# OettlM/STEDM

Hardware: AMD Instinct MI355X
Metric: U-Net denoising steps/sec (32x32x4 latent, bs=64) (higher is better)
Workload: dtype f16; 1 GPU; HER2-style DDIM-50 + CFG 1.5 (rescale 0.7) denoising step, NS32 U-Net (234.6M params, random-init PRNG weights), 32x32x4 latents + 3-ch layout concat, style vector 512; batch_per_gpu=64, global_batch=64, latent=32x32x4, cfg=cond+uncond per step, parallelism=dp1 (independent latents, no in-loop collective)

## Files before the change

include/stedm_hip.h:

```cpp
#ifndef STEDM_HIP_H
#define STEDM_HIP_H

#include <stdint.h>

#ifdef __cplusplus
extern "C" {
#endif

#define STEDM_ABI_VERSION 12

#define STEDM_F16 0
#define STEDM_BF16 1

#define STEDM_CONV_S1 0
#define STEDM_CONV_DOWN 1
#define STEDM_CONV_UP 2
#define STEDM_CONV_UP_SUBPIXEL 3
#define STEDM_CONV_S2D 4

int stedm_abi_version(void);
const char* stedm_last_error(void);
int stedm_device_cus(void);

#define STEDM_F16G_RAW 1
// ... 90 lines not shown
  int32_t gn_only;
  void* gn_out16_lo;
  void* qkv_q;
  void* qkv_k;
  void* qkv_vt;
  int32_t qkv_T, qkv_Tp, qkv_heads;
  float qkv_qscale;
  const float* ln_gamma;
  const float* ln_beta;
  const float* ln_res;
  float ln_eps;
  int32_t out16_stride;
  void* gn_coop;
  const uint32_t* gn_coop_epoch;
  uint32_t* gn_coop_tmo;
} stedm_conv_args;
int stedm_conv_igemm(const stedm_conv_args* args, void* stream);
int stedm_conv_fused_skip_ok(const stedm_conv_args* args);
int stedm_conv3x3_tiles_ok(int Hout, int Wout);
int stedm_im2col_rows16(const void* src16, void* dst16, int B, int Hs, int Ws, int C, int mode, void* stream);
int stedm_conv_rs_ok(const stedm_conv_args* args);

int stedm_conv_in(const float* x1, int c1, const float* x2, int c2, int x2_bmod, const float* w_oihw,
                  const float* bias, float* out, int B, int H, int W, int cout, float* chan_stats, void* stream);
int stedm_conv_out(const float* src, int c, const float* chan_stats, int nslab, const float* gamma, const float* beta,
                   float eps, int groups, const float* w_hwio, const float* bias, float* out, int B, int H, int W,
                   int cout, void* stream);

int stedm_time_embed(const int64_t* t, const float* freqs, const float* w0t, const float* b0,
                     const float* w2t, const float* b2, float* emb, float* ws, int B, int mc, int ted,
// ... 135 lines not shown
```

stedm_amd/_lib.py:

```python
from __future__ import annotations

import ctypes as C
import os

_HERE = os.path.dirname(os.path.abspath(__file__))
LIB_PATH = os.environ.get("STEDM_HIP_LIB") or os.path.join(_HERE, "libstedm_hip.so")

ABI_VERSION = 12
F16, BF16 = 0, 1
CONV_S1, CONV_DOWN, CONV_UP, CONV_UP_SUBPIXEL, CONV_S2D = 0, 1, 2, 3, 4


class StedmHipError(RuntimeError):
    pass


class ConvArgs(C.Structure):
    _fields_ = [
        ("src1", C.c_void_p), ("src2", C.c_void_p),
        ("c1", C.c_int32), ("c2", C.c_int32), ("src2_bmod", C.c_int32),
        ("B", C.c_int32), ("Hin", C.c_int32), ("Win", C.c_int32),
        ("mode", C.c_int32), ("ks", C.c_int32),
        ("scale", C.c_void_p), ("shift", C.c_void_p),
        ("act", C.c_int32),
# ... 1 lines not shown
        ("emb", C.c_void_p), ("emb_bstride", C.c_int32),
        ("res", C.c_void_p), ("out", C.c_void_p),
        ("cout", C.c_int32), ("npass", C.c_int32), ("mm_dtype", C.c_int32),
        ("src16_hi", C.c_void_p), ("src16_lo", C.c_void_p),
        ("act_out", C.c_int32), ("out16_hi", C.c_void_p), ("out16_lo", C.c_void_p),
        ("w_frag", C.c_void_p), ("chan_stats", C.c_void_p),
        ("src16b_hi", C.c_void_p), ("w_frag_b", C.c_void_p), ("bias_b", C.c_void_p), ("cb", C.c_int32),
        ("ws", C.c_void_p), ("ws_floats", C.c_int64), ("chan_nslab", C.c_int32), ("w_frag16", C.c_void_p), ("w_frag_b16", C.c_void_p), ("pad_br", C.c_int32),
        ("gn_gamma", C.c_void_p), ("gn_beta", C.c_void_p), ("gn_eps", C.c_float), ("gn_groups", C.c_int32), ("gn_act", C.c_int32), ("gn_out16", C.c_void_p), ("gn_mr", C.c_void_p), ("gn_only", C.c_int32),
        ("gn_out16_lo", C.c_void_p),
        ("qkv_q", C.c_void_p), ("qkv_k", C.c_void_p), ("qkv_vt", C.c_void_p),
        ("qkv_T", C.c_int32), ("qkv_Tp", C.c_int32), ("qkv_heads", C.c_int32), ("qkv_qscale", C.c_float),
        ("ln_gamma", C.c_void_p), ("ln_beta", C.c_void_p), ("ln_res", C.c_void_p), ("ln_eps", C.c_float),
        ("out16_stride", C.c_int32),
        ("gn_coop", C.c_void_p), ("gn_coop_epoch", C.c_void_p), ("gn_coop_tmo", C.c_void_p),
    ]


_P, _I, _F = C.c_void_p, C.c_int, C.c_float
SIGNATURES = {
    "stedm_abi_version": (_I, []),
    "stedm_last_error": (C.c_char_p, []),
    "stedm_device_cus": (_I, []),
    "stedm_f16_guard_set": (_I, [_P]),
    "stedm_pack_conv_weight": (_I, [_P, _P, _P, _I, _I, _I, _I, _P]),
    "stedm_pack_conv_weight_up": (_I, [_P, _P, _P, _I, _I, _I, _P]),
    "stedm_pack_conv_weight_frag": (_I, [_P, _P, _I, _I, _I, _I, _P]),
    "stedm_pack_conv_weight_up_frag": (_I, [_P, _P, _I, _I, _I, _P]),
    "stedm_pack_conv_weight_frag16": (_I, [_P, C.c_long, C.c_long, _I, _P, _I, _I, _I, _I, _P]),
    "stedm_pack_conv_weight_frag16_hl": (_I, [_P, C.c_long, C.c_long, _I, _P, _I, _I, _I, _P]),
# ... 133 lines not shown
```

stedm_amd/csrc/conv_dma_bf16_p1.hip:

```cpp
#include "conv_igemm_dma9.inc"
#include "conv_rs.inc"
namespace stedm {
int conv_dma_pick_bf16_p1(ConvParams& p, hipStream_t st, bool dry) {
  int rc = conv_rs_pick<__bf16>(p, st, dry);
  if (rc >= 0 || dry || p.a.src16b_hi || p.a.mode == STEDM_CONV_S2D || p.a.qkv_q || p.a.ln_gamma) return rc;
  rc = dma9_pick<__bf16>(p, st);
  return rc >= 0 ? rc : dma_pick<1, __bf16>(p, st);
}
}

extern "C" int stedm_debug_conv_stamps(unsigned long long* host_out, int nblocks) {
  if (!host_out || nblocks <= 0 || nblocks > 2048) { stedm::set_error("debug_conv_stamps: bad args"); return 1; }
  hipError_t e = hipMemcpyFromSymbol(host_out, HIP_SYMBOL(g_conv_stamps), (size_t)nblocks * 8 * sizeof(unsigned long long));
  if (e != hipSuccess) { stedm::set_error("debug_conv_stamps: %s", hipGetErrorString(e)); return 2; }
  return 0;
}
```

stedm_amd/csrc/conv_dma_f16_p1.hip:

```cpp
#include "conv_igemm_dma9.inc"
#include "conv_rs.inc"
namespace stedm {
int conv_dma_pick_f16_p1(ConvParams& p, hipStream_t st, bool dry) {
  int rc = conv_rs_pick<_Float16>(p, st, dry);
  if (rc >= 0 || dry || p.a.src16b_hi || p.a.mode == STEDM_CONV_S2D || p.a.qkv_q || p.a.ln_gamma) return rc;
  rc = dma9_pick<_Float16>(p, st);
  return rc >= 0 ? rc : dma_pick<1, _Float16>(p, st);
}
}
```

stedm_amd/csrc/conv_igemm.hip:

```cpp
#include <stdlib.h>

#include "conv_common.hpp"
using namespace stedm;

constexpr int BM = 128, NTHREADS = 256;

template <int BKC, int NPASS, typename T>
__global__ void __launch_bounds__(NTHREADS, 2) conv_igemm_kernel(const ConvParams p) {
  using V8 = typename MM<T>::V8;
  using V4 = typename MM<T>::V4;
  constexpr int AST = BKC * 2 + 16;
  constexpr int BST = BKC * 2 + 16;
  constexpr int NPL = NPASS == 3 ? 2 : 1;
  constexpr int QC = BKC / 4;
  constexpr int POSL = NTHREADS / QC;
  constexpr int PCS = BKC / 8;
  constexpr int BPT = BN * PCS / NTHREADS;
  constexpr int KSTEPS = BKC / 16;

  extern __shared__ __attribute__((aligned(16))) unsigned char smem[];
  unsigned char* sA = smem;
  const int a_plane = p.NP * AST;
  unsigned char* sB = smem + NPL * a_plane;
  constexpr int b_plane = BN * BST;
// ... 368 lines not shown
  } else if (a.mode == STEDM_CONV_DOWN) {
    STEDM_CHECK_ARG(a.Hin % 2 == 0 && a.Win % 2 == 0, "conv_igemm: stride-2 needs even Hin/Win");
    p.Hout = a.Hin / 2; p.Wout = a.Win / 2;
  } else if (a.mode == STEDM_CONV_UP) {
    p.Hout = a.Hin * 2; p.Wout = a.Win * 2;
  } else {
    p.Hout = a.Hin; p.Wout = a.Win;
  }
  p.HWout = p.Hout * p.Wout;
  p.M = a.B * p.HWout;
  STEDM_CHECK_ARG(p.Cin % 32 == 0 && (a.c2 == 0 || a.c1 % 32 == 0),
                  "conv_igemm: channel counts must be multiples of 32 (c1=%d c2=%d)", a.c1, a.c2);
  STEDM_CHECK_ARG(!a.src16b_hi || (a.src16_hi && !a.src1 && ((a.w_frag && a.w_frag_b) || (a.w_frag16 && a.w_frag_b16)) && a.ks == 3 && a.mode == STEDM_CONV_S1 && a.npass == 1 && !a.res &&
                                   a.cb > 0 && a.cb % 64 == 0),
                  "conv_igemm: the fused skip phase needs the DMA path (src16 only), 3x3 stride 1, single product, w_frag + w_frag_b, cb %% 64 == 0, no res");
  return 0;
}

static int conv_dispatch(ConvParams& p, void* stream) {
  const stedm_conv_args& a = p.a;
  { const int rc = conv_setup(p); if (rc) return rc; }
  hipStream_t st = as_stream(stream);
  static const int dbg0 = getenv("STEDM_CONV_DBG") ? atoi(getenv("STEDM_CONV_DBG")) : 0;
#ifdef STEDM_CONV_DIAG
  p.dbg = dbg0;
#else
  p.dbg = 0;
  if (dbg0) { set_error("conv_igemm: STEDM_CONV_DBG=%d needs a diagnostic build (tools/conv_diag.sh, STEDM_HIP_LIB); the shipped kernels compile no ablation switch", dbg0); return 1; }
#endif
  p.ovf = a.mm_dtype == STEDM_F16 ? f16_guard_flag() : nullptr;
// ... 12 lines not shown
```

stedm_amd/csrc/conv_igemm_dma.hip:

```cpp
#include "conv_common.hpp"
using namespace stedm;

namespace stedm {
int conv_dma_pick_f16_p1(ConvParams&, hipStream_t, bool dry);
int conv_dma_pick_f16_p3(ConvParams&, hipStream_t, bool dry);
int conv_dma_pick_bf16_p1(ConvParams&, hipStream_t, bool dry);
int conv_dma_pick_bf16_p3(ConvParams&, hipStream_t, bool dry);
}

int stedm::conv_launch_dma(ConvParams& p, hipStream_t st, bool dry) {
  const stedm_conv_args& a = p.a;
  if (a.src16b_hi && a.npass != 1) { set_error("conv_igemm(dma): the fused skip phase is single-product only"); return 1; }
  if (dry && a.npass != 1 && !a.w_frag16) return 1;
  if (a.src16b_hi && ((long)a.B * a.Hin * a.Win * a.cb >= (1L << 31) || a.cb * 2 + 256 > STEDM_ZERO_PAGE_BYTES)) {
    set_error("conv_igemm(dma): fused skip operand too large (cb=%d)", a.cb);
    return 1;
  }
  if ((long)a.B * a.Hin * a.Win * p.Cin >= (1L << 31)) {
    set_error("conv_igemm(dma): activation tensor too large for 32-bit element offsets");
    return 1;
  }
  if (p.Cin * 2 + 256 > STEDM_ZERO_PAGE_BYTES) { set_error("conv_igemm(dma): Cin too large for the zero page"); return 1; }
  const bool f16 = a.mm_dtype == STEDM_F16;
  int rc = a.npass == 3 ? (f16 ? conv_dma_pick_f16_p3(p, st, dry) : conv_dma_pick_bf16_p3(p, st, dry))
                        : (f16 ? conv_dma_pick_f16_p1(p, st, dry) : conv_dma_pick_bf16_p1(p, st, dry));
  if (dry) return rc < 0 ? 1 : 0;
  if (rc < 0 && a.ln_gamma) { set_error("conv_igemm(dma): the register-streamed kernel does not run this LayerNorm-epilogue problem (see stedm_conv_rs_ok)"); return 1; }
  if (rc < 0 && a.qkv_q) { set_error("conv_igemm(dma): the register-streamed kernel does not run this qkv-epilogue problem (see stedm_conv_rs_ok)"); return 1; }
  if (rc < 0 && a.src16b_hi) { set_error("conv_igemm(dma): no kernel runs this fused skip problem (see stedm_conv_fused_skip_ok)"); return 1; }
  if (rc < 0) { set_error("conv_igemm(dma): no tile configuration fits (Hin=%d Win=%d mode=%d Cin=%d)", a.Hin, a.Win, a.mode, p.Cin); return 1; }
  return rc;
}
```

stedm_amd/csrc/conv_rs.inc:

```
#pragma once
#include <type_traits>

#include "conv_igemm_dma.inc"

static __device__ unsigned long long g_conv_stamps[2048 * 8];
#define STAMP(K) if (STEDM_DBG(p.dbg, 1024) && tid == 0 && blockIdx.x < 2048) g_conv_stamps[blockIdx.x * 8 + (K)] = wall_clock64()
#define STAMPC(K) if (STEDM_DBG(p.dbg, 1024) && tid == 0 && blockIdx.x < 2048) g_conv_stamps[blockIdx.x * 8 + (K)] = __builtin_amdgcn_s_memtime()

#ifdef STEDM_CONV_DIAG
#define RS_DIAG(BIT) ((STEDM_CONV_DIAG) & (BIT))
#else
#define RS_DIAG(BIT) 0
#endif

__device__ __forceinline__ float rs_lane_xor1(float v) {
  return __builtin_bit_cast(float, __builtin_amdgcn_mov_dpp(__builtin_bit_cast(int, v), 0xB1, 0xF, 0xF, true));
}
template <typename T>
__device__ __forceinline__ unsigned rs_pack2(float lo, float hi) {
  typedef T V2T __attribute__((ext_vector_type(2)));
  V2T v; v[0] = (T)lo; v[1] = (T)hi;
  return __builtin_bit_cast(unsigned, v);
}

// ... 404 lines not shown
    const bool okm = m < p.M;
    if (SUBPIX && !s2d && okm) {
      const int rem = m - b * p.HWout, y = div_w(rem), x = rem - y * p.Wout;
      m = (b * 2 * p.Hout + 2 * y + py) * (2 * p.Wout) + 2 * x + px;
    }
    sM[ml] = okm ? m : -1;
    sMb[ml] = b;
  }
  }
  if (is_loader) {
    bool early[3] = {false, false, false};
#define WAIT_VM(N) asm volatile("s_waitcnt vmcnt(" #N ")" ::: "memory")
    const int aw = wave - NCW;
    const uint16_t* a_hi = reinterpret_cast<const uint16_t*>(a.src16_hi);
    const uint16_t* zero16 = reinterpret_cast<const uint16_t*>(g_zero_page);
    const int nslots = (nai + 1 - aw) / 2;
    constexpr int MAXS = IS1X1 ? 16 : 13;
    const uint16_t* asrc[MAXS];
    const int lpos = lane / CPP, lphys = lane % CPP;
    const long lo_delta = P3 ? reinterpret_cast<const uint16_t*>(a.src16_lo) - a_hi : 0;
    unsigned zmask = 0;
#define LO_SRC(K) (asrc[K] + (((zmask >> (K)) & 1u) ? 0 : lo_delta))
#pragma unroll
    for (int k = 0; k < MAXS; ++k) {
      asrc[k] = zero16;
      if (k < nslots) {
        const int pos = (aw + 2 * k) * PPI + lpos;
        const int logical = M16 ? lphys : lphys ^ ((pos / RPB) % CPP);
        const int pix = patch_pixel(pos);
        asrc[k] = (pix >= 0 ? a_hi + (long)pix * p.Cin : zero16) + logical * 8;
        if (P3 && pix < 0) zmask |= 1u << k;
        if (!STEDM_DBG(p.dbg, 2)) {
#pragma unroll
          for (int pl = 0; pl < NPL; ++pl) {
            GLDS16(asrc[k] + (cbeg * NPL + pl) * (BROW / 2), sA + pl * (a_plane + pl_skew) + (aw + 2 * k) * 1024);
            if (P3) GLDS16(LO_SRC(k) + (cbeg * NPL + pl) * (BROW / 2), sA + a_half + pl * (a_plane + pl_skew) + (aw + 2 * k) * 1024);
          }
        }
      }
    }
    auto issue_a = [&](int chunk) {
      if STEDM_DBG(p.dbg, 2) return;
      unsigned char* dsta = sA + (chunk % NABUF) * a_buf;
#pragma unroll
      for (int pl = 0; pl < NPL; ++pl) {
// ... 506 lines not shown
  const int nsub = BMT / rows_per;
  unsigned bad16 = 0u, badn = 0u;
  for (int sub = 0; sub < nsub; ++sub) {
    float cs[4] = {0.f, 0.f, 0.f, 0.f}, cq[4] = {0.f, 0.f, 0.f, 0.f};
    const bool only16 = !a.out && a.out16_hi && !a.out16_lo;
    const bool fast = vec_ok && !split && (a.out ? !a.out16_hi : only16) && !a.act_out && !(ragged && a.emb);
    if (active && fast) {
      float ev[4] = {0.f, 0.f, 0.f, 0.f};
      const int rfirst = sub * rows_per;
      if (a.emb && sM[rfirst] >= 0) {
        const float* ep = a.emb + (long)sMb[rfirst] * a.emb_bstride + n;
#pragma unroll
        for (int u = 0; u < 4; ++u) ev[u] = ep[u];
      }
      const bool has_emb = a.emb != nullptr;
      const float* __restrict__ resp = a.res;
      float* __restrict__ outp = a.out;
      typedef T V4T16 __attribute__((ext_vector_type(4)));
      T* __restrict__ o16p = only16 ? reinterpret_cast<T*>(a.out16_hi) : nullptr;
      const long ostr16 = a.out16_stride ? a.out16_stride : a.cout;
      constexpr int RB = 8;
      for (int row0 = rfirst + rg; row0 < rfirst + rows_per; row0 += RB * (NT / 32)) {
        int mm[RB];
        float4 r4[RB];
#pragma unroll
        for (int k = 0; k < RB; ++k) {
          const int row = row0 + k * (NT / 32);
          mm[k] = row < rfirst + rows_per ? sM[row] : -1;
          r4[k] = make_float4(0.f, 0.f, 0.f, 0.f);
          if (resp && mm[k] >= 0) r4[k] = *reinterpret_cast<const float4*>(resp + (long)mm[k] * a.cout + n);
        }
// ... 24 lines not shown
      for (int row = sub * rows_per + rg; row < (sub + 1) * rows_per; row += NT / 32) {
        const int m = sM[row];
        if (m < 0) continue;
        const float4 v4 = *reinterpret_cast<const float4*>(sStage + row * SST + c4 * 4);
        float v[4] = {v4.x + bv[0], v4.y + bv[1], v4.z + bv[2], v4.w + bv[3]};
        const long o = (long)m * a.cout + n;
        if (split) {
          *reinterpret_cast<float4*>(a.ws + (long)kz * p.M * ((SUBPIX && !s2d) ? 4 : 1) * a.cout + o) = v4;
          continue;
        }
        if (a.emb) {
          const float* ep = a.emb + (long)sMb[row] * a.emb_bstride + n;
          for (int u = 0; u < nv; ++u) v[u] += ep[u];
        }
        if (a.res) {
          if (vec_ok) { const float4 r4 = *reinterpret_cast<const float4*>(a.res + o); v[0] += r4.x; v[1] += r4.y; v[2] += r4.z; v[3] += r4.w; }
          else for (int u = 0; u < nv; ++u) v[u] += a.res[o + u];
        }
        if (a.act_out == 2) {
#pragma unroll
          for (int u = 0; u < 4; ++u) v[u] = gelu_erf_f(v[u]);
        }
        if (a.out) {
          if (vec_ok) *reinterpret_cast<float4*>(a.out + o) = make_float4(v[0], v[1], v[2], v[3]);
          else for (int u = 0; u < nv; ++u) a.out[o + u] = v[u];
        }
        if (a.out16_hi) {
          typedef T V4T __attribute__((ext_vector_type(4)));
          if (vec_ok) {
            V4T h4, l4;
#pragma unroll
            for (int u = 0; u < 4; ++u) { h4[u] = (T)v[u]; l4[u] = (T)(v[u] - (float)h4[u]); }
// ... 166 lines not shown
      const float4 e4 = *reinterpret_cast<const float4*>(a.emb + (long)b * a.emb_bstride + n);
      add.x += e4.x; add.y += e4.y; add.z += e4.z; add.w += e4.w;
    }
#pragma unroll 2
    for (int pix = px0 + tp; pix < px1; pix += npl) {
      const long o = ((long)b * HW + pix) * C + n;
      float4 pz[KSMAX];
#pragma unroll
      for (int z = 0; z < KSMAX; ++z)
        if (KSMAX == 2 || z < ksplit) pz[z] = *reinterpret_cast<const float4*>(a.ws + z * plane + o);
      float4 v = pz[0];
#pragma unroll
      for (int z = 1; z < KSMAX; ++z)
        if (KSMAX == 2 || z < ksplit) { v.x += pz[z].x; v.y += pz[z].y; v.z += pz[z].z; v.w += pz[z].w; }
      v.x += add.x; v.y += add.y; v.z += add.z; v.w += add.w;
      if (a.res) { const float4 r4 = *reinterpret_cast<const float4*>(a.res + o); v.x += r4.x; v.y += r4.y; v.z += r4.z; v.w += r4.w; }
      if (GN || a.out) *reinterpret_cast<float4*>(a.out + o) = v;
      if (a.out16_hi) {
        const long o16 = a.out16_stride ? ((long)b * HW + pix) * a.out16_stride + n : o;
        if (a.mm_dtype == STEDM_F16) {
          f16x4 h4; h4[0] = (_Float16)v.x; h4[1] = (_Float16)v.y; h4[2] = (_Float16)v.z; h4[3] = (_Float16)v.w;
          *reinterpret_cast<f16x4*>(reinterpret_cast<_Float16*>(a.out16_hi) + o16) = h4;
          bad16 |= f16_over_v4<_Float16>(h4);
        } else {
          bf16x4 h4; h4[0] = (__bf16)v.x; h4[1] = (__bf16)v.y; h4[2] = (__bf16)v.z; h4[3] = (__bf16)v.w;
          *reinterpret_cast<bf16x4*>(reinterpret_cast<__bf16*>(a.out16_hi) + o16) = h4;
        }
      }
      s[0] += v.x; s[1] += v.y; s[2] += v.z; s[3] += v.w;
      q[0] += v.x * v.x; q[1] += v.y * v.y; q[2] += v.z * v.z; q[3] += v.w * v.w;
    }
// ... 190 lines not shown
    else conv_splitk_reduce_kernel<16><<<grid, 256, 0, st>>>(ra, HWo, plane, kp.ksplit, qbs, p.ovf, slab_px);
    STEDM_LAUNCH_CHECK();
    stats = ra.chan_stats != nullptr;
  }
  if (stats) p.stats_done = 1;
  if (p.gn_tile || p.gn_coop) p.gn_done = 1;
  return 0;
}

template <typename T>
static int conv_rs_pick(ConvParams& p, hipStream_t st, bool dry = false) {
  const stedm_conv_args& a = p.a;
  const bool fuse = a.src16b_hi != nullptr;
  if (fuse && (a.ks != 3 || a.mode != STEDM_CONV_S1 || !a.w_frag_b || a.cb <= 0 || a.cb % 64 != 0 || a.res)) return -1;
  if ((!a.w_frag && !a.w_frag16) || (a.act_out != 0 && a.act_out != 2) || a.npass != 1 || a.mode == STEDM_CONV_DOWN) return -1;
  const bool s2d = a.mode == STEDM_CONV_S2D;
  const bool sp = (a.mode == STEDM_CONV_UP_SUBPIXEL || s2d) && p.taps == 4 && p.Cin % 32 == 0;
  if (s2d && !sp) return -1;
  const bool k3 = a.ks == 3 && p.taps == 9 && p.Cin % 16 == 0, k1 = a.ks == 1 && p.Cin % 64 == 0;
  if (!k3 && !k1 && !sp) return -1;
  if (a.qkv_q && (!k1 || fuse || !a.w_frag)) return -1;
  if (a.ln_gamma && (!k1 || fuse || !a.w_frag || a.cout > 128)) return -1;
  static int cus = 0;
  if (cus == 0) { cus = stedm_device_cus(); if (cus <= 0) cus = 256; }
  ConvParams q = p;
  if (!conv_geometry(q, 256, true)) return -1;
  q.ksplit = 0;
  auto pick_split = [&](long tiles, int nchunks, int planes = 1, int nchunks2 = 0) {
    if (!a.ws || (!a.out && !a.out16_hi) || a.out16_lo || a.act_out || a.cout % 4 != 0 || (a.emb && a.emb_bstride % 4 != 0) || a.ln_gamma || a.qkv_q) return 0;
    const int minc = tiles * 16 <= cus ? 1 : (tiles * 8 <= cus ? 2 : 4);
// ... 25 lines not shown
  if (fuse) {
    if (!k3) return -1;
    int rc = m16 ? conv_rs_try<T, 4, RS_3X3M, true>(p, q, st, dry) : -1;
    if (rc >= 0 || !a.w_frag || !a.w_frag_b) return rc;
    if (m16) q.ksplit = 0;
    return conv_rs_try<T, 4, RS_3X3, true>(p, q, st, dry);
  }
  if (sp) {
    if (subm) { const int rc = conv_rs_try<T, 4, RS_SUBM>(p, q, st, dry); if (rc >= 0 || !a.w_frag) return rc; }
    return a.w_frag ? conv_rs_try<T, 4, RS_SUB>(p, q, st, dry) : -1;
  }
  if (k1) {
    const int rc = conv_rs_try<T, 4, RS_1X1N>(p, q, st, dry);
    return rc >= 0 ? rc : conv_rs_try<T, 4, RS_1X1>(p, q, st, dry);
  }
  if (m16) { const int rc = conv_rs_try<T, 4, RS_3X3M>(p, q, st, dry); if (rc >= 0 || !a.w_frag) return rc; q.ksplit = 0; }
  return conv_rs_try<T, 4, RS_3X3>(p, q, st, dry);
}

template <typename T>
static int conv_rs3_pick(ConvParams& p, hipStream_t st, bool dry = false) {
  const stedm_conv_args& a = p.a;
  const bool k1 = a.ks == 1 && p.taps == 1;
  const bool s2d = a.mode == STEDM_CONV_S2D;
  const bool sp = (a.mode == STEDM_CONV_UP_SUBPIXEL || s2d) && a.ks == 3 && p.taps == 4;
  if (a.npass != 3 || !a.w_frag16 || !a.src16_lo || a.src16b_hi || !(sp || ((k1 || (a.ks == 3 && p.taps == 9)) && a.mode == STEDM_CONV_S1)) ||
      p.Cin % 32 != 0 || p.Cin < (k1 ? 64 : 128) || (a.act_out != 0 && a.act_out != 2))
    return -1;
  static int cus = 0;
  if (cus == 0) { cus = stedm_device_cus(); if (cus <= 0) cus = 256; }
  ConvParams q = p;
// ... 20 lines not shown
```

stedm_amd/ops.py:

```python
from __future__ import annotations

import ctypes as C
from dataclasses import dataclass
from typing import Optional, Tuple

import torch

from . import _lib
from ._lib import BF16, CONV_DOWN, CONV_S1, CONV_S2D, CONV_UP, CONV_UP_SUBPIXEL, F16, ConvArgs, check, lib


@dataclass(frozen=True)
class Precision:
    mm_dtype: int = F16
    npass: int = 3
    attn_fp8: bool = False

    @staticmethod
    def parse(name: str) -> "Precision":
        table = {"parity": Precision(F16, 3), "parity_bf16": Precision(BF16, 3),
                 "fast": Precision(F16, 1), "f16": Precision(F16, 1), "bf16": Precision(BF16, 1),
                 "fp8": Precision(BF16, 1, True), "bf16+fp8attn": Precision(BF16, 1, True)}
        if name not in table:
            raise ValueError(f"unknown precision {name!r}; choose from {sorted(table)}")
# ... 408 lines not shown
    return conv_igemm(None, w_hi.view(cout, 1, 9 * C), None if w_lo is None else w_lo.view(cout, 1, 9 * C), out, prec=prec, ks=1, mode=CONV_S1,
                      src16=(cols[0], cols[1]), **kw)


def conv_igemm(src1: Optional[torch.Tensor], w_hi: torch.Tensor, w_lo: Optional[torch.Tensor], out: torch.Tensor, *, prec: Precision,
               ks: int = 3, mode: int = CONV_S1, src2: Optional[torch.Tensor] = None, src2_bmod: int = 0,
               scale: Optional[torch.Tensor] = None, shift: Optional[torch.Tensor] = None, act: int = 0,
               bias: Optional[torch.Tensor] = None, emb: Optional[torch.Tensor] = None, emb_offset: int = 0,
               emb_bstride: int = 0, res: Optional[torch.Tensor] = None,
               src16: Optional[Tuple[torch.Tensor, Optional[torch.Tensor]]] = None, act_out: int = 0,
               out16: Optional[Tuple[torch.Tensor, Optional[torch.Tensor]]] = None, w_frag: Optional[torch.Tensor] = None,
               chan_stats: Optional[torch.Tensor] = None,
               skip: Optional[Tuple[torch.Tensor, torch.Tensor, Optional[torch.Tensor]]] = None, query_fused: bool = False, query_rs: bool = False,
               ws: Optional[torch.Tensor] = None, pad_br: bool = False, w_frag16: Optional[torch.Tensor] = None,
               gn_next: Optional[tuple] = None, qkv_planes: Optional[tuple] = None, ln_after: Optional[tuple] = None, coop: Optional[tuple] = None,
               out16_stride: int = 0, cout: Optional[int] = None):
    if src16 is not None and src1 is None and ks == 3 and mode in (CONV_S1, CONV_DOWN, CONV_UP) and not out16_stride:
        _, H_, W_, _ = src16[0].shape
        Ho_, Wo_ = ((H_ - 1) // 2 + 1, (W_ - 1) // 2 + 1) if mode == CONV_DOWN else ((2 * H_, 2 * W_) if mode == CONV_UP else (H_, W_))
        if not conv3x3_tiles_ok(Ho_, Wo_):
            if query_fused or query_rs:
                return False
            return _conv3x3_generic(src16, w_hi, w_lo, out, prec=prec, mode=mode, scale=scale, shift=shift, act=act, bias=bias, emb=emb,
                                    emb_offset=emb_offset, emb_bstride=emb_bstride, res=res, act_out=act_out, out16=out16, chan_stats=chan_stats,
                                    skip=skip, ws=ws, gn_next=gn_next)
    if out is not None:
        _chk(out, name="out")
    a = ConvArgs()
    a.act_out = act_out
    if gn_next is not None:
        g_w, g_b, g_eps, g_groups, g_act, g_out = gn_next[:6]
        g_lo = None
# ... 57 lines not shown
        a.qkv_T, a.qkv_Tp, a.qkv_heads, a.qkv_qscale = int(qT), int(qTp), int(qH), float(qs)
        oshape = (1, 1, src16[0].shape[2], 3 * int(qH) * 64)
    else:
        oshape = out.shape if out is not None else out16[0].shape
        if cout is not None:
            oshape = tuple(oshape[:-1]) + (int(cout),)
    if src1 is not None:
        _chk(src1, name="src1")
        B, Hin, Win, c1 = src1.shape
        a.src1 = src1.data_ptr()
        a.src2 = _ptr(src2)
        c2 = 0 if src2 is None else src2.shape[-1]
    else:
        B, Hin, Win, c1 = src16[0].shape
        c2 = 0
    if src16 is not None:
        assert src16[0].dtype == torch.int16 and src16[0].is_contiguous() and tuple(src16[0].shape) == (B, Hin, Win, c1 + c2)
        a.src16_hi = src16[0].data_ptr()
        a.src16_lo = _ptr(src16[1]) if prec.npass == 3 else None
    a.c1, a.c2, a.src2_bmod = c1, c2, src2_bmod
    a.B, a.Hin, a.Win = B, Hin, Win
    a.mode, a.ks = mode, ks
    a.scale, a.shift, a.act = _ptr(scale), _ptr(shift), act
    lazy = w_hi if isinstance(w_hi, LazyPlanes) else None
    if lazy is not None:
        w_hi, w_lo = lazy._val if lazy._val is not None else (w_frag if w_frag is not None else w_frag16, None)
    a.w_hi, a.w_lo = _ptr(w_hi), (_ptr(w_lo) if prec.npass == 3 else None)
    a.bias = _ptr(bias)
    a.emb = None if emb is None else emb.data_ptr() + 4 * emb_offset
    a.emb_bstride = emb_bstride
    a.res = _ptr(res)
    a.out = _ptr(out)
    a.cout = oshape[-1]
    a.npass, a.mm_dtype = prec.npass, prec.mm_dtype
    if lazy is not None and lazy._val is None:
        if src16 is None or (w_frag is None and w_frag16 is None) or prec.npass != 1 or not lib().stedm_conv_rs_ok(C.byref(a)):
            w_hi, w_lo = lazy.get()
            a.w_hi, a.w_lo = _ptr(w_hi), (_ptr(w_lo) if prec.npass == 3 else None)
    elif mode == CONV_UP_SUBPIXEL:
        assert w_hi.shape == (4 * a.cout, 4, a.c1 + a.c2), (w_hi.shape, a.cout, a.c1, a.c2)
    elif mode == CONV_S2D:
        assert w_hi is None and (w_frag is not None or w_frag16 is not None) and src1 is None, \
            "the space-to-depth form runs on the register-streamed kernel only"
    else:
        assert w_hi.shape == (a.cout, ks * ks, a.c1 + a.c2), (w_hi.shape, a.cout, ks, a.c1, a.c2)
    if query_fused:
# ... 601 lines not shown
```

stedm_amd/unet.py:

```python
from __future__ import annotations

import math
import os
from typing import Dict, List, Optional, Tuple

import torch
import torch.nn as nn

from . import ops
from ._lib import BF16, F16, CONV_S2D, CONV_DOWN, CONV_S1, CONV_UP, CONV_UP_SUBPIXEL, StedmHipError
from .ops import Precision


def zero_module(module: nn.Module) -> nn.Module:
    for p in module.parameters():
        p.detach().zero_()
    return module


class GroupNorm32(nn.GroupNorm):
    """util.py:214-216 (container; eps 1e-5, 32 groups)."""


class TimestepBlock(nn.Module):
# ... 415 lines not shown
        if not (prec.npass == 1 and co == 128 and 256 < H * W <= 1024 and B * H * W // 256 >= ops.device_cus() and not os.environ.get("STEDM_NO_GN_COOP")):
            return None
        ck = (site, B)
        words = self._coop_bufs.get(ck)
        if words is None:
            words = self._coop_bufs[ck] = torch.zeros((B, 4, 128, 2), dtype=torch.int64, device=self._coop_state.device)
        if not self._coop_advanced:
            ops.step_advance(self._coop_state, 1)
            self._coop_advanced = True
        return words, self._coop_state

    def _cat_plane(self, B, H, W, co, next_cat):
        self._catpp ^= 1
        return self._buf(f"cat16.{self._catpp}.{B}x{H}x{W}x{next_cat}", (B, H, W, next_cat), torch.int16)

    def _res(self, tag: str, rb: ResBlock, x1, x2, emb_all, emb_off, emb_bstride, x2_bmod=0, want16=False, next_cat=None, next_norm=None):
        prec = self.precision
        B, H, W, _ = x1.shape
        co = rb.out_channels
        dma = self.conv_path == "dma"
        pk = self._packed[id(rb.in_layers[2])]
        h = self._buf(tag + ".h" if self._tape is not None else f"h.{B}x{H}x{W}x{co}", (B, H, W, co))
        self._last_h = h
        has_skip = not isinstance(rb.skip_connection, nn.Identity)
        h16_next = gn_next = None
        if dma:
            if has_skip:
                a16, x16 = self._norm16(rb.in_layers[0], 1, x1, x2, x2_bmod, want_raw=True)
            else:
                a16 = self._norm16(rb.in_layers[0], 1, x1, x2, x2_bmod)
# ... 17 lines not shown
            coop_runs = coop is not None
            if (gn_next is not None and self._tape is None and prec.npass == 1 and prec.mm_dtype == BF16 and H * W > 256 and B >= 8 and not coop_runs and
                    not os.environ.get("STEDM_NO_H16ONLY") and ops.gn_apply16c_x16_ok(co, 0, gn2.num_groups)):
                kw1 = dict(prec=prec, src16=a16, bias=pk.bias, emb=emb_all, emb_offset=emb_off, emb_bstride=emb_bstride, w_frag=pk.frag,
                           chan_stats=self._cs_new(h), ws=ws, w_frag16=pk.frag16)
                hraw = self._buf(f"h16raw.{B}x{H}x{W}x{co}", (B, H, W, co), torch.int16)
                key1 = ("h16only", id(rb), B, H, W)
                ok1 = self._consts.get(key1)
                if ok1 is None:
                    ok1 = bool(ops.conv_igemm(None, pk.hi, pk.lo, None, query_rs=True, out16=(hraw, None), out16_stride=co, cout=co, **kw1))
                    self._consts[key1] = ok1
                if ok1:
                    ops.conv_igemm(None, pk.hi, pk.lo, None, out16=(hraw, None), out16_stride=co, cout=co, **kw1)
                    ops.gn_apply16c_x16(co, self._cs[h.data_ptr()], None, None, h16_next[0], hraw, prec, gn2.weight, gn2.bias, gn2.eps, gn2.num_groups, 1)
                    done1 = True
            if not done1:
                ops.conv_igemm(None, pk.hi, pk.lo, h, prec=prec, src16=a16, bias=pk.bias, emb=emb_all, emb_offset=emb_off,
                               emb_bstride=emb_bstride, w_frag=pk.frag, chan_stats=self._cs_new(h), ws=ws, w_frag16=pk.frag16, gn_next=gn_next,
                               coop=coop)
        else:
            sc, sh = self._gn(tag + ".gn1", rb.in_layers[0], x1, x2, x2_bmod)
            ops.conv_igemm(x1, pk.hi, pk.lo, h, prec=prec, src2=x2, src2_bmod=x2_bmod, scale=sc, shift=sh, act=1, bias=pk.bias,
                           emb=emb_all, emb_offset=emb_off, emb_bstride=emb_bstride)
        out = self._buf(tag + ".out", (B, H, W, co))
        pk2 = self._packed[id(rb.out_layers[3])]
        o16 = None
        if dma and want16:
            o16 = self._planes(B, H, W, co, "up16")
            self._raw16[out.data_ptr()] = o16
        gnn, npl, coop2 = None, None, None
# ... 348 lines not shown
```

Before: 166.5 steps/s.

## Split concat ResBlock conv to compute shared skip half once across CFG batch

For decoder ResBlocks whose input is a concat of x1 and a skip tensor shared across CFG halves (x2_bmod), the first 3x3 conv is split along input channels. The skip-channel portion runs only on the Bs unique rows into a partial buffer, and the main conv over the remaining channels adds it back via a new modulo-B residual addend. Input channel windows are read through a new src16_stride field. This is meant to avoid recomputing the skip-channel GEMM for duplicated batch rows. The cost is an extra kernel launch and a partial buffer write/read, and the path is limited to small spatial sizes with the register-streamed kernel.

Result: faster. 169.7 steps/s (median of 6 runs) (+2.0%).

```diff
diff --git a/include/stedm_hip.h b/include/stedm_hip.h
--- a/include/stedm_hip.h
+++ b/include/stedm_hip.h
@@ -7,7 +7,7 @@
 extern "C" {
 #endif
 
-#define STEDM_ABI_VERSION 12
+#define STEDM_ABI_VERSION 13
 
 #define STEDM_F16 0
 #define STEDM_BF16 1
@@ -128,6 +128,8 @@
   void* gn_coop;
   const uint32_t* gn_coop_epoch;
   uint32_t* gn_coop_tmo;
+  int32_t src16_stride;
+  int32_t res_bmod;
 } stedm_conv_args;
 int stedm_conv_igemm(const stedm_conv_args* args, void* stream);
 int stedm_conv_fused_skip_ok(const stedm_conv_args* args);
diff --git a/stedm_amd/_lib.py b/stedm_amd/_lib.py
--- a/stedm_amd/_lib.py
+++ b/stedm_amd/_lib.py
@@ -6,7 +6,7 @@
 _HERE = os.path.dirname(os.path.abspath(__file__))
 LIB_PATH = os.environ.get("STEDM_HIP_LIB") or os.path.join(_HERE, "libstedm_hip.so")
 
-ABI_VERSION = 12
+ABI_VERSION = 13
 F16, BF16 = 0, 1
 CONV_S1, CONV_DOWN, CONV_UP, CONV_UP_SUBPIXEL, CONV_S2D = 0, 1, 2, 3, 4
 
@@ -39,6 +39,7 @@
         ("ln_gamma", C.c_void_p), ("ln_beta", C.c_void_p), ("ln_res", C.c_void_p), ("ln_eps", C.c_float),
         ("out16_stride", C.c_int32),
         ("gn_coop", C.c_void_p), ("gn_coop_epoch", C.c_void_p), ("gn_coop_tmo", C.c_void_p),
+        ("src16_stride", C.c_int32), ("res_bmod", C.c_int32),
     ]
 
 
diff --git a/stedm_amd/csrc/conv_dma_bf16_p1.hip b/stedm_amd/csrc/conv_dma_bf16_p1.hip
--- a/stedm_amd/csrc/conv_dma_bf16_p1.hip
+++ b/stedm_amd/csrc/conv_dma_bf16_p1.hip
@@ -3,7 +3,8 @@
 namespace stedm {
 int conv_dma_pick_bf16_p1(ConvParams& p, hipStream_t st, bool dry) {
   int rc = conv_rs_pick<__bf16>(p, st, dry);
-  if (rc >= 0 || dry || p.a.src16b_hi || p.a.mode == STEDM_CONV_S2D || p.a.qkv_q || p.a.ln_gamma) return rc;
+  if (rc >= 0 || dry || p.a.src16b_hi || p.a.mode == STEDM_CONV_S2D || p.a.qkv_q || p.a.ln_gamma || p.a.src16_stride || p.a.res_bmod)
+    return rc;
   rc = dma9_pick<__bf16>(p, st);
   return rc >= 0 ? rc : dma_pick<1, __bf16>(p, st);
 }
diff --git a/stedm_amd/csrc/conv_dma_f16_p1.hip b/stedm_amd/csrc/conv_dma_f16_p1.hip
--- a/stedm_amd/csrc/conv_dma_f16_p1.hip
+++ b/stedm_amd/csrc/conv_dma_f16_p1.hip
@@ -3,7 +3,8 @@
 namespace stedm {
 int conv_dma_pick_f16_p1(ConvParams& p, hipStream_t st, bool dry) {
   int rc = conv_rs_pick<_Float16>(p, st, dry);
-  if (rc >= 0 || dry || p.a.src16b_hi || p.a.mode == STEDM_CONV_S2D || p.a.qkv_q || p.a.ln_gamma) return rc;
+  if (rc >= 0 || dry || p.a.src16b_hi || p.a.mode == STEDM_CONV_S2D || p.a.qkv_q || p.a.ln_gamma || p.a.src16_stride || p.a.res_bmod)
+    return rc;
   rc = dma9_pick<_Float16>(p, st);
   return rc >= 0 ? rc : dma_pick<1, _Float16>(p, st);
 }
diff --git a/stedm_amd/csrc/conv_igemm.hip b/stedm_amd/csrc/conv_igemm.hip
--- a/stedm_amd/csrc/conv_igemm.hip
+++ b/stedm_amd/csrc/conv_igemm.hip
@@ -406,6 +406,13 @@
   STEDM_CHECK_ARG(!a.src16b_hi || (a.src16_hi && !a.src1 && ((a.w_frag && a.w_frag_b) || (a.w_frag16 && a.w_frag_b16)) && a.ks == 3 && a.mode == STEDM_CONV_S1 && a.npass == 1 && !a.res &&
                                    a.cb > 0 && a.cb % 64 == 0),
                   "conv_igemm: the fused skip phase needs the DMA path (src16 only), 3x3 stride 1, single product, w_frag + w_frag_b, cb %% 64 == 0, no res");
+  STEDM_CHECK_ARG(a.src16_stride == 0 || (a.src16_hi && !a.src1 && a.src16_stride >= p.Cin && a.src16_stride % 8 == 0 && ((uintptr_t)a.src16_hi & 15) == 0),
+                  "conv_igemm: src16_stride needs the DMA path (src16 only), a 16-B aligned src16_hi and a stride >= c1 + c2, a multiple of 8 (stride %d, Cin %d)",
+                  a.src16_stride, p.Cin);
+  STEDM_CHECK_ARG(a.res_bmod == 0 || (a.res && a.res_bmod > 0 && a.res_bmod <= a.B),
+                  "conv_igemm: res_bmod needs res and 0 < res_bmod <= B (res_bmod %d, B %d)", a.res_bmod, a.B);
+  STEDM_CHECK_ARG((a.src16_stride == 0 && a.res_bmod == 0) || (a.src16_hi && !a.src1 && a.npass == 1 && a.ks == 3 && a.mode == STEDM_CONV_S1 && a.w_frag16 && !a.src16b_hi),
+                  "conv_igemm: src16_stride / res_bmod need a single-product 3x3 stride-1 problem with w_frag16 and no fused skip phase");
   return 0;
 }
 
diff --git a/stedm_amd/csrc/conv_igemm_dma.hip b/stedm_amd/csrc/conv_igemm_dma.hip
--- a/stedm_amd/csrc/conv_igemm_dma.hip
+++ b/stedm_amd/csrc/conv_igemm_dma.hip
@@ -16,7 +16,7 @@
     set_error("conv_igemm(dma): fused skip operand too large (cb=%d)", a.cb);
     return 1;
   }
-  if ((long)a.B * a.Hin * a.Win * p.Cin >= (1L << 31)) {
+  if ((long)a.B * a.Hin * a.Win * (a.src16_stride > p.Cin ? a.src16_stride : p.Cin) >= (1L << 31)) {
     set_error("conv_igemm(dma): activation tensor too large for 32-bit element offsets");
     return 1;
   }
@@ -27,6 +27,11 @@
   if (dry) return rc < 0 ? 1 : 0;
   if (rc < 0 && a.ln_gamma) { set_error("conv_igemm(dma): the register-streamed kernel does not run this LayerNorm-epilogue problem (see stedm_conv_rs_ok)"); return 1; }
   if (rc < 0 && a.qkv_q) { set_error("conv_igemm(dma): the register-streamed kernel does not run this qkv-epilogue problem (see stedm_conv_rs_ok)"); return 1; }
+  if (rc < 0 && (a.src16_stride || a.res_bmod)) {
+    set_error("conv_igemm(dma): no kernel runs this channel-window / modulo-B addend problem (src16_stride %d, res_bmod %d; see stedm_conv_rs_ok)",
+              a.src16_stride, a.res_bmod);
+    return 1;
+  }
   if (rc < 0 && a.src16b_hi) { set_error("conv_igemm(dma): no kernel runs this fused skip problem (see stedm_conv_fused_skip_ok)"); return 1; }
   if (rc < 0) { set_error("conv_igemm(dma): no tile configuration fits (Hin=%d Win=%d mode=%d Cin=%d)", a.Hin, a.Win, a.mode, p.Cin); return 1; }
   return rc;
diff --git a/stedm_amd/csrc/conv_rs.inc b/stedm_amd/csrc/conv_rs.inc
--- a/stedm_amd/csrc/conv_rs.inc
+++ b/stedm_amd/csrc/conv_rs.inc
@@ -442,6 +442,7 @@
     const int aw = wave - NCW;
     const uint16_t* a_hi = reinterpret_cast<const uint16_t*>(a.src16_hi);
     const uint16_t* zero16 = reinterpret_cast<const uint16_t*>(g_zero_page);
+    const long apix = a.src16_stride ? a.src16_stride : p.Cin;
     const int nslots = (nai + 1 - aw) / 2;
     constexpr int MAXS = IS1X1 ? 16 : 13;
     const uint16_t* asrc[MAXS];
@@ -456,7 +457,7 @@
         const int pos = (aw + 2 * k) * PPI + lpos;
         const int logical = M16 ? lphys : lphys ^ ((pos / RPB) % CPP);
         const int pix = patch_pixel(pos);
-        asrc[k] = (pix >= 0 ? a_hi + (long)pix * p.Cin : zero16) + logical * 8;
+        asrc[k] = (pix >= 0 ? a_hi + (long)pix * apix : zero16) + logical * 8;
         if (P3 && pix < 0) zmask |= 1u << k;
         if (!STEDM_DBG(p.dbg, 2)) {
 #pragma unroll
@@ -993,7 +994,8 @@
         for (int u = 0; u < 4; ++u) ev[u] = ep[u];
       }
       const bool has_emb = a.emb != nullptr;
-      const float* __restrict__ resp = a.res;
+      const float* __restrict__ resp = (a.res && a.res_bmod && sM[rfirst] >= 0)
+                                           ? a.res - (long)(sMb[rfirst] - sMb[rfirst] % a.res_bmod) * p.HWout * a.cout : a.res;
       float* __restrict__ outp = a.out;
       typedef T V4T16 __attribute__((ext_vector_type(4)));
       T* __restrict__ o16p = only16 ? reinterpret_cast<T*>(a.out16_hi) : nullptr;
@@ -1048,8 +1050,9 @@
           for (int u = 0; u < nv; ++u) v[u] += ep[u];
         }
         if (a.res) {
-          if (vec_ok) { const float4 r4 = *reinterpret_cast<const float4*>(a.res + o); v[0] += r4.x; v[1] += r4.y; v[2] += r4.z; v[3] += r4.w; }
-          else for (int u = 0; u < nv; ++u) v[u] += a.res[o + u];
+          const long orr = a.res_bmod ? o - (long)(sMb[row] - sMb[row] % a.res_bmod) * p.HWout * a.cout : o;
+          if (vec_ok) { const float4 r4 = *reinterpret_cast<const float4*>(a.res + orr); v[0] += r4.x; v[1] += r4.y; v[2] += r4.z; v[3] += r4.w; }
+          else for (int u = 0; u < nv; ++u) v[u] += a.res[orr + u];
         }
         if (a.act_out == 2) {
 #pragma unroll
@@ -1246,7 +1249,10 @@
       for (int z = 1; z < KSMAX; ++z)
         if (KSMAX == 2 || z < ksplit) { v.x += pz[z].x; v.y += pz[z].y; v.z += pz[z].z; v.w += pz[z].w; }
       v.x += add.x; v.y += add.y; v.z += add.z; v.w += add.w;
-      if (a.res) { const float4 r4 = *reinterpret_cast<const float4*>(a.res + o); v.x += r4.x; v.y += r4.y; v.z += r4.z; v.w += r4.w; }
+      if (a.res) {
+        const long orr = a.res_bmod ? o - (long)(b - b % a.res_bmod) * HW * C : o;
+        const float4 r4 = *reinterpret_cast<const float4*>(a.res + orr); v.x += r4.x; v.y += r4.y; v.z += r4.z; v.w += r4.w;
+      }
       if (GN || a.out) *reinterpret_cast<float4*>(a.out + o) = v;
       if (a.out16_hi) {
         const long o16 = a.out16_stride ? ((long)b * HW + pix) * a.out16_stride + n : o;
@@ -1467,6 +1473,8 @@
   const bool fuse = a.src16b_hi != nullptr;
   if (fuse && (a.ks != 3 || a.mode != STEDM_CONV_S1 || !a.w_frag_b || a.cb <= 0 || a.cb % 64 != 0 || a.res)) return -1;
   if ((!a.w_frag && !a.w_frag16) || (a.act_out != 0 && a.act_out != 2) || a.npass != 1 || a.mode == STEDM_CONV_DOWN) return -1;
+  const bool win = a.src16_stride != 0 || a.res_bmod != 0;
+  if (win && (fuse || a.ks != 3 || a.mode != STEDM_CONV_S1 || !a.w_frag16 || a.qkv_q || a.ln_gamma)) return -1;
   const bool s2d = a.mode == STEDM_CONV_S2D;
   const bool sp = (a.mode == STEDM_CONV_UP_SUBPIXEL || s2d) && p.taps == 4 && p.Cin % 32 == 0;
   if (s2d && !sp) return -1;
@@ -1522,7 +1530,8 @@
     const int rc = conv_rs_try<T, 4, RS_1X1N>(p, q, st, dry);
     return rc >= 0 ? rc : conv_rs_try<T, 4, RS_1X1>(p, q, st, dry);
   }
-  if (m16) { const int rc = conv_rs_try<T, 4, RS_3X3M>(p, q, st, dry); if (rc >= 0 || !a.w_frag) return rc; q.ksplit = 0; }
+  if (win && !m16) return -1;
+  if (m16) { const int rc = conv_rs_try<T, 4, RS_3X3M>(p, q, st, dry); if (rc >= 0 || !a.w_frag || win) return rc; q.ksplit = 0; }
   return conv_rs_try<T, 4, RS_3X3>(p, q, st, dry);
 }
 
diff --git a/stedm_amd/ops.py b/stedm_amd/ops.py
--- a/stedm_amd/ops.py
+++ b/stedm_amd/ops.py
@@ -446,8 +446,10 @@
                skip: Optional[Tuple[torch.Tensor, torch.Tensor, Optional[torch.Tensor]]] = None, query_fused: bool = False, query_rs: bool = False,
                ws: Optional[torch.Tensor] = None, pad_br: bool = False, w_frag16: Optional[torch.Tensor] = None,
                gn_next: Optional[tuple] = None, qkv_planes: Optional[tuple] = None, ln_after: Optional[tuple] = None, coop: Optional[tuple] = None,
-               out16_stride: int = 0, cout: Optional[int] = None):
-    if src16 is not None and src1 is None and ks == 3 and mode in (CONV_S1, CONV_DOWN, CONV_UP) and not out16_stride:
+               out16_stride: int = 0, cout: Optional[int] = None, src16_chans: Optional[Tuple[int, int]] = None, rows: Optional[int] = None,
+               res_bmod: int = 0):
+    if (src16 is not None and src1 is None and ks == 3 and mode in (CONV_S1, CONV_DOWN, CONV_UP) and not out16_stride and src16_chans is None and
+            not res_bmod):
         _, H_, W_, _ = src16[0].shape
         Ho_, Wo_ = ((H_ - 1) // 2 + 1, (W_ - 1) // 2 + 1) if mode == CONV_DOWN else ((2 * H_, 2 * W_) if mode == CONV_UP else (H_, W_))
         if not conv3x3_tiles_ok(Ho_, Wo_):
@@ -535,9 +537,20 @@
     else:
         B, Hin, Win, c1 = src16[0].shape
         c2 = 0
+    ch0 = 0
+    if src16_chans is not None or rows is not None:
+        assert src1 is None and prec.npass == 1
+        cw = src16_chans if src16_chans is not None else (0, c1)
+        assert 0 <= cw[0] < cw[1] <= src16[0].shape[-1] and cw[0] % 8 == 0, cw
+        ch0, c1 = int(cw[0]), int(cw[1] - cw[0])
+        if rows is not None:
+            assert 0 < rows <= src16[0].shape[0]
+            B = int(rows)
+        a.src16_stride = src16[0].shape[-1]
     if src16 is not None:
-        assert src16[0].dtype == torch.int16 and src16[0].is_contiguous() and tuple(src16[0].shape) == (B, Hin, Win, c1 + c2)
-        a.src16_hi = src16[0].data_ptr()
+        assert src16[0].dtype == torch.int16 and src16[0].is_contiguous() and tuple(src16[0].shape[1:]) == (Hin, Win, ch0 + c1 + c2 if not a.src16_stride else a.src16_stride)
+        assert a.src16_stride or src16[0].shape[0] == B
+        a.src16_hi = src16[0].data_ptr() + 2 * ch0
         a.src16_lo = _ptr(src16[1]) if prec.npass == 3 else None
     a.c1, a.c2, a.src2_bmod = c1, c2, src2_bmod
     a.B, a.Hin, a.Win = B, Hin, Win
@@ -551,6 +564,9 @@
     a.emb = None if emb is None else emb.data_ptr() + 4 * emb_offset
     a.emb_bstride = emb_bstride
     a.res = _ptr(res)
+    if res_bmod:
+        assert res is not None and res.shape[0] == res_bmod
+        a.res_bmod = int(res_bmod)
     a.out = _ptr(out)
     a.cout = oshape[-1]
     a.npass, a.mm_dtype = prec.npass, prec.mm_dtype
diff --git a/stedm_amd/unet.py b/stedm_amd/unet.py
--- a/stedm_amd/unet.py
+++ b/stedm_amd/unet.py
@@ -453,6 +453,50 @@
         self._catpp ^= 1
         return self._buf(f"cat16.{self._catpp}.{B}x{H}x{W}x{next_cat}", (B, H, W, next_cat), torch.int16)
 
+    SKIP_SHARE_MIN_FLOP = 5.0e10
+
+    def _skip_share(self, rb: ResBlock, x1, x2, plane):
+        prec = self.precision
+        H, W = plane.shape[1], plane.shape[2]
+        if (x2 is None or self._tape is not None or self.conv_path != "dma" or prec.npass != 1 or H * W > 256 or
+                os.environ.get("STEDM_NO_CFG_SKIP_SHARE") or not ops.conv3x3_tiles_ok(H, W)):
+            return None
+        conv = rb.in_layers[2]
+        pk = self._packed[id(conv)]
+        Bs, c_h, C, co = x2.shape[0], x1.shape[-1], x1.shape[-1] + x2.shape[-1], rb.out_channels
+        key = ("skipshare", id(rb), Bs, H, W, c_h, C)
+        if key in self._consts:
+            return self._consts[key]
+        got = None
+        gw = C // rb.in_layers[0].num_groups
+        s0 = -(-(-(-c_h // gw) * gw) // 32) * 32
+        if pk.frag16 is not None and C % gw == 0:
+            part = self._buf(f"skp.{Bs}x{H}x{W}x{co}", (Bs, H, W, co))
+            ws = self._skip_ws(Bs, H, W, co)
+            probe = torch.empty((1, 1, 1, 1), dtype=torch.int16, device=part.device)
+            def rs_ok(chans, res):
+                return ops.conv_igemm(None, ops.LazyPlanes(lambda: (probe, None)), None, part, prec=prec, src16=(plane, None), src16_chans=chans,
+                                      rows=Bs, w_frag16=probe, ws=ws, res=res, res_bmod=Bs if res is not None else 0, query_rs=True)
+            while C - s0 >= 256 and 2.0 * Bs * H * W * co * (C - s0) * 9 >= self.SKIP_SHARE_MIN_FLOP:
+                if rs_ok((s0, C), None) and rs_ok((0, s0), part):
+                    break
+                s0 += 32
+            else:
+                s0 = C
+            if s0 < C and s0 >= 256:
+                w = conv.weight.detach().float()
+
+                def no_planes():
+                    raise StedmHipError("the split concat convolution runs on the register-streamed kernel only")
+                got = (s0, (ops.LazyPlanes(no_planes), ops.pack_conv_weight_frag16(w[:, :s0].contiguous(), prec)),
+                       (ops.LazyPlanes(no_planes), ops.pack_conv_weight_frag16(w[:, s0:].contiguous(), prec)))
+        self._consts[key] = got
+        return got
+
+    def _skip_ws(self, Bs, H, W, co):
+        nel = Bs * H * W * co
+        return self._buf("conv_ws", ((16 if nel <= (1 << 20) else (4 if nel <= (1 << 22) else 2)) * nel,)) if nel <= (1 << 23) else None
+
     def _res(self, tag: str, rb: ResBlock, x1, x2, emb_all, emb_off, emb_bstride, x2_bmod=0, want16=False, next_cat=None, next_norm=None):
         prec = self.precision
         B, H, W, _ = x1.shape
@@ -500,6 +544,17 @@
                     ops.conv_igemm(None, pk.hi, pk.lo, None, out16=(hraw, None), out16_stride=co, cout=co, **kw1)
                     ops.gn_apply16c_x16(co, self._cs[h.data_ptr()], None, None, h16_next[0], hraw, prec, gn2.weight, gn2.bias, gn2.eps, gn2.num_groups, 1)
                     done1 = True
+            share = self._skip_share(rb, x1, x2, a16[0]) if not done1 else None
+            if share is not None:
+                s0, (ha, fa), (hb, fb) = share
+                Bs, C = x2.shape[0], a16[0].shape[-1]
+                part = self._buf(f"skp.{Bs}x{H}x{W}x{co}", (Bs, H, W, co))
+                ops.conv_igemm(None, hb, None, part, prec=prec, src16=(a16[0], None), src16_chans=(s0, C), rows=Bs, w_frag16=fb,
+                               ws=self._skip_ws(Bs, H, W, co))
+                ops.conv_igemm(None, ha, None, h, prec=prec, src16=(a16[0], None), src16_chans=(0, s0), bias=pk.bias, emb=emb_all,
+                               emb_offset=emb_off, emb_bstride=emb_bstride, res=part, res_bmod=Bs, chan_stats=self._cs_new(h), ws=ws,
+                               w_frag16=fa, gn_next=gn_next, coop=coop)
+                done1 = True
             if not done1:
                 ops.conv_igemm(None, pk.hi, pk.lo, h, prec=prec, src16=a16, bias=pk.bias, emb=emb_all, emb_offset=emb_off,
                                emb_bstride=emb_bstride, w_frag=pk.frag, chan_stats=self._cs_new(h), ws=ws, w_frag16=pk.frag16, gn_next=gn_next,
```
